# Desperodoo/distributed_multi_agent_reinforcement_learning

Hardware: AMD Instinct MI355X
Metric: env-steps/sec (whole node), pursuit-evasion 8-agent 4096-env (higher is better)
Workload: dtype f64 environment / f32 policy (f32 matrix products evaluated from exact 3-way bf16 operand splits, f32 accumulation and storage)

## Files before the change

### distributed_multi_agent_reinforcement_learning_amd/csrc/mappo_ops.hip

```cpp
#include <hip/hip_runtime.h>
#include <stdint.h>
#include <stdlib.h>
#include <string.h>

#include <mutex>

#include "mappo_ops.h"
#include "mappo_ops_diag.h"
#include "sb_common.hpp"
#include "sb_wgrad.hpp"
#include "ppo_diag.hpp"

namespace {

constexpr int MAX_P = 16;

__device__ __forceinline__ float msg_dot4(const float *w, const float4 &qv) {
    return __builtin_fmaf(w[3], qv.w, __builtin_fmaf(w[2], qv.z, __builtin_fmaf(w[1], qv.y, w[0] * qv.x)));
}

struct MsgDims {
    int R, P, K, E, din, q_div, adj_mode, rpb;
    int64_t p_rs, q_rs, e_rs, adj_rs, o_is;
};
// ... 2165 lines not shown
    if (pt == 4) MSGW3_PT(4) else if (pt == 8) MSGW3_PT(8) else MSGW3_PT(16)
#undef MSGW3_PT
#undef MSGW3_LAUNCH
#undef MSGW3_LAUNCH1
    return (int)hipGetLastError();
}

}

#include "gauss_policy.hpp"
#include "imitation.hpp"
#include "value_norm.hpp"
#include "fused_adam.hpp"

constexpr int SB_WGRAD_WGS = 256;

static bool sb_wgrad_shape_ok(int M, int N) {
    return (M == 128 || M == 256 || M == 384) && (N == 128 || N == 256 || N == 384) && M + N <= 512 && M * N < 256 * 256;
}

template <int MT, int NT>
int launch_sb_wgrad(int64_t K, const float *A, int64_t lda, const float *B, int64_t ldb, float *Cm, int accumulate, float *part, hipStream_t st,
                    const float *A2 = nullptr, int64_t lda2 = 0, int M1 = 0) {
    using C = SbWgCfg<MT, NT>;
    static std::once_flag once;
    static hipError_t attr_rc = hipSuccess;
    std::call_once(once, [] { attr_rc = hipFuncSetAttribute((const void *)k_sb_wgrad<MT, NT>, hipFuncAttributeMaxDynamicSharedMemorySize, C::LDS_BYTES); });
    if (attr_rc != hipSuccess) return (int)attr_rc;
    hipLaunchKernelGGL((k_sb_wgrad<MT, NT>), dim3(SB_WGRAD_WGS), dim3(SB_WG_THREADS), C::LDS_BYTES, st, A, lda, B, ldb, K, part, A2, lda2, M1);
    hipLaunchKernelGGL(k_wgrad_reduce, dim3((C::M * C::N + 63) / 64), dim3(256), 0, st, SB_WGRAD_WGS, C::M * C::N, (const float *)part, Cm, accumulate);
    return (int)hipGetLastError();
}

extern "C" {

int dhgn_msg_agg_fwd(int32_t R, int32_t P, int32_t K, int32_t E, int32_t din, const float *p, int64_t p_rs, const float *q,
                     int64_t q_rs, int32_t q_div, const float *e, int64_t e_rs, const void *adj, int64_t adj_rs, int32_t adj_mode,
                     const int32_t *kvalid, const float *W, const float *b, float *out, int64_t out_stride, void *stream) {
    int rc = check_msg(R, P, K, E, din, q_div, adj_mode, adj, kvalid, e);
    if (rc) return rc;
    if (R == 0) return 0;
    if ((q_rs & 3) || out_stride < E) return MO_ERR_BAD_ARG;
    int grid;
    const MsgDims d = msg_dims(R, P, K, E, din, q_div, adj_mode, p_rs, q_rs, e_rs, adj_rs, out_stride, FWD_BLOCKS, &grid);
    const bool qs = msg_q_small(K), as = msg_adj_small(P, K, adj_mode), ev2 = (E % 128) == 0;
#define MSGW_FWD1(PT, QS, AS, EV) hipLaunchKernelGGL((k_msgw_fwd<PT, QS, AS, EV>), dim3(grid), dim3(E / EV), 0, (hipStream_t)stream, d, p, q, e, adj, kvalid, W, b, out)
#define MSGW_FWD(PT, QS, AS) do { if (ev2) MSGW_FWD1(PT, QS, AS, 2); else MSGW_FWD1(PT, QS, AS, 1); } while (0)
#define MSGW_FWD_PT(PT) { if (qs && as) MSGW_FWD(PT, true, true); else if (qs) MSGW_FWD(PT, true, false); else if (as) MSGW_FWD(PT, false, true); else MSGW_FWD(PT, false, false); }
    if (P <= 8) MSGW_FWD_PT(8) else MSGW_FWD_PT(16)
#undef MSGW_FWD_PT
#undef MSGW_FWD
#undef MSGW_FWD1
    return (int)hipGetLastError();
}

int dhgn_msg_agg3_fwd(const mo_msg_rel *rel, int32_t R, int32_t P, int32_t E, const float *p, int64_t p_rs, float *out, int64_t out_stride,
                      void *stream) {
    if (!rel || !p || !out || R < 0) return MO_ERR_BAD_ARG;
    if (R == 0) return 0;
    return launch_msgw3(rel, R, P, E, p, p_rs, rel[2].kvalid, out, nullptr, 0, out_stride, stream, false);
}

int dhgn_msg_agg3_pair_fwd(const mo_msg_rel *rel, int32_t R, int32_t P, int32_t E, const float *p, int64_t p_rs, const int32_t *o_kvalid,
                           float *out_actor, float *out_critic, int64_t out_stride, void *stream) {
    if (!rel || !p || !out_actor || !out_critic || R < 0) return MO_ERR_BAD_ARG;
    if (R == 0) return 0;
// ... 340 lines not shown
}

int64_t wgrad_split_workspace(int32_t M, int32_t N) {
    if (!sb_wgrad_shape_ok(M, N)) return -1;
    return (int64_t)SB_WGRAD_WGS * M * N * sizeof(float);
}

int wgrad_split_tn(int64_t K, int32_t M, int32_t N, const float *A, int64_t lda, const float *B, int64_t ldb, float *C, int32_t accumulate,
                   void *workspace, void *stream) {
    if (K < 1 || !sb_wgrad_shape_ok(M, N) || !A || !B || !C || !workspace) return MO_ERR_BAD_ARG;
    if (lda < M || ldb < N || (lda & 3) || (ldb & 3) || ((uintptr_t)A & 15) || ((uintptr_t)B & 15)) return MO_ERR_BAD_ARG;
    hipStream_t st = (hipStream_t)stream;
    float *part = (float *)workspace;
#define SB_WG(mt, nt) if (M == 128 * mt && N == 128 * nt) return launch_sb_wgrad<mt, nt>(K, A, lda, B, ldb, C, accumulate, part, st);
    SB_WG(1, 1) SB_WG(1, 2) SB_WG(2, 1) SB_WG(1, 3) SB_WG(3, 1)
#undef SB_WG
    return MO_ERR_BAD_ARG;
}

int wgrad_split_tn2(int64_t K, int32_t M1, int32_t M2, int32_t N, const float *A1, int64_t lda1, const float *A2, int64_t lda2, const float *B, int64_t ldb,
                    float *C, int32_t accumulate, void *workspace, void *stream) {
    const int M = M1 + M2;
    if (K < 1 || M1 < 4 || M2 < 4 || (M1 & 3) || (M2 & 3) || !sb_wgrad_shape_ok(M, N) || !A1 || !A2 || !B || !C || !workspace) return MO_ERR_BAD_ARG;
    if (lda1 < M1 || lda2 < M2 || ldb < N || (lda1 & 3) || (lda2 & 3) || (ldb & 3) || ((uintptr_t)A1 & 15) || ((uintptr_t)A2 & 15) || ((uintptr_t)B & 15))
        return MO_ERR_BAD_ARG;
    hipStream_t st = (hipStream_t)stream;
    float *part = (float *)workspace;
#define SB_WG(mt, nt) if (M == 128 * mt && N == 128 * nt) return launch_sb_wgrad<mt, nt>(K, A1, lda1, B, ldb, C, accumulate, part, st, A2, lda2, M1);
    SB_WG(1, 1) SB_WG(1, 2) SB_WG(2, 1) SB_WG(1, 3) SB_WG(3, 1)
#undef SB_WG
    return MO_ERR_BAD_ARG;
}

int fcra_neighbour_mean(int32_t R, int32_t P, int32_t E, int32_t T, const float *z_actor, int64_t za_episode_stride, int64_t za_step_stride,
                        const float *z_critic, int64_t zc_episode_stride, int64_t zc_step_stride, const float *adj, int64_t adj_row_stride,
                        const float *bias, int32_t relu, float *out_actor, float *out_critic, int64_t out_stride, void *stream) {
    const mo_nbr_job job{z_actor, z_critic, bias, out_actor, out_critic};
    return fcra_neighbour_mean_multi(1, &job, R, P, E, T, za_episode_stride, za_step_stride, zc_episode_stride, zc_step_stride, adj, adj_row_stride, relu,
                                     out_stride, stream);
}

int fcra_neighbour_mean_multi(int32_t n_jobs, const mo_nbr_job *jobs, int32_t R, int32_t P, int32_t E, int32_t T, int64_t za_episode_stride,
                              int64_t za_step_stride, int64_t zc_episode_stride, int64_t zc_step_stride, const float *adj, int64_t adj_row_stride,
                              int32_t relu, int64_t out_stride, void *stream) {
    if (n_jobs < 1 || n_jobs > MO_NBR_MAX_JOBS || !jobs) return MO_ERR_BAD_ARG;
    if (R < 0 || P < 1 || P > MAX_P || E < 64 || E > 1024 || (E & 63) || T < 1 || (R % T) || out_stride < E) return MO_ERR_BAD_ARG;
    NbrJobs a_jobs;
    memset(&a_jobs, 0, sizeof a_jobs);
    for (int k = 0; k < n_jobs; k++) {
        const mo_nbr_job &m = jobs[k];
        if ((m.out_actor && (!m.z_actor || !adj)) || (m.out_critic && !m.z_critic) || (!m.out_actor && !m.out_critic)) return MO_ERR_BAD_ARG;
        a_jobs.j[k] = m;
    }
    if (R == 0) return 0;
    NbrArgs a{R, P, E, T, relu, za_episode_stride, za_step_stride, zc_episode_stride, zc_step_stride, adj_row_stride, out_stride};
    if (E == 128 && P <= 8 && !(out_stride & 3) && !(za_episode_stride & 3) && !(za_step_stride & 3) && !(zc_episode_stride & 3) && !(zc_step_stride & 3)) {
        bool aligned = true;
        for (int k = 0; k < n_jobs; k++) {
            const mo_nbr_job &m = jobs[k];
            aligned = aligned && !(((uintptr_t)m.z_actor | (uintptr_t)m.z_critic | (uintptr_t)m.bias | (uintptr_t)m.out_actor | (uintptr_t)m.out_critic) & 15);
        }
        if (aligned) {
            const int per4 = 4096 / n_jobs, blocks = (R + 3) / 4;
            hipLaunchKernelGGL(k_nbr_mean4, dim3(blocks < per4 ? blocks : per4, n_jobs), dim3(256), 0, (hipStream_t)stream, a, a_jobs, adj);
            return (int)hipGetLastError();
        }
// ... 178 lines not shown
```

### distributed_multi_agent_reinforcement_learning_amd/csrc/sb_wgrad.hpp

```cpp
#pragma once
#include "sb_common.hpp"

constexpr int SB_WG_MMA_WAVES = 8, SB_WG_LOAD_WAVES = 4, SB_WG_THREADS = 64 * (SB_WG_MMA_WAVES + SB_WG_LOAD_WAVES);

template <int MT, int NT>
struct SbWgCfg {
    static constexpr int M = 128 * MT, N = 128 * NT, COLS = M + N, FQ = COLS / 4;
    static constexpr int CR = 16, NO = 2;
    static constexpr int WGM = MT >= NT ? 4 : 2;
    static constexpr int WGN = 8 / WGM;
    static constexpr int TM = M / 32 / WGM, TN = N / 32 / WGN;
    static constexpr int UNITS = 2 * NO * FQ;
    static constexpr int LT = 64 * SB_WG_LOAD_WAVES;
    static constexpr int UL = (UNITS + LT - 1) / LT;
    static constexpr int DEPTH = UL == 1 ? 4 : 3;
    static constexpr int IMG = 3 * NO * COLS;
    static constexpr int LDS_BYTES = 2 * IMG * 16;
};

__device__ __forceinline__ int sb_swz(int f) { return (f & ~3) | ((f & 3) ^ ((f >> 3) & 3)); }

template <int MT, int NT>
__device__ __forceinline__ void sb_wgrad_loader(int lw, int lane, const float *__restrict__ A, int64_t lda, const float *__restrict__ B, int64_t ldb, int64_t K,
                                                const float *__restrict__ A2, int64_t lda2, int M1, int64_t c_beg, int64_t c_end, bool tail,
                                                uint4 *sb_lds) {
    using C = SbWgCfg<MT, NT>;
    const float *src[C::UL];
    int64_t ld[C::UL];
    bool on[C::UL];
    int row_in_chunk[C::UL], slot2[C::UL], sx[C::UL];
#pragma unroll
    for (int u = 0; u < C::UL; u++) {
        const int unit = 64 * lw + lane + C::LT * u;
        on[u] = (u + 1) * C::LT <= C::UNITS || 64 * lw + C::LT * u < C::UNITS;
        const int rest = on[u] ? unit / C::FQ : 0, col = on[u] ? 4 * (unit % C::FQ) : 0;
        row_in_chunk[u] = 4 * rest;
        const bool in_a2 = A2 != nullptr && col >= M1 && col < C::M;
        ld[u] = in_a2 ? lda2 : (col < C::M ? lda : ldb);
        src[u] = (in_a2 ? A2 + (col - M1) : (col < C::M ? A + col : B + (col - C::M))) + row_in_chunk[u] * ld[u];
        slot2[u] = 2 * ((rest >> 1) * C::COLS + col) + (rest & 1);
        sx[u] = (col >> 3) & 3;
    }
    constexpr int D = C::DEPTH;
    float4 raw[D][C::UL][4];
    auto fetch = [&](float4 (&r)[C::UL][4], int64_t c) {
        c = c < c_end ? c : c_end - 1;
#pragma unroll
        for (int u = 0; u < C::UL; u++) {
            const float *p = src[u] + c * C::CR * ld[u];
#pragma unroll
            for (int j = 0; j < 4; j++) r[u][j] = *(const float4 *)(p + j * ld[u]);
        }
    };
    auto stage = [&](const float4 (&r)[C::UL][4], uint4 *img) {
        uint2 *img2 = (uint2 *)img;
#pragma unroll
        for (int u = 0; u < C::UL; u++) {
            if (!on[u]) continue;
#pragma unroll
            for (int t = 0; t < 4; t++) {
                uint32_t p[3][2];
#pragma unroll
                for (int q = 0; q < 2; q++) {
                    const float4 &v0 = r[u][2 * q], &v1 = r[u][2 * q + 1];
                    const float x0 = t == 0 ? v0.x : t == 1 ? v0.y : t == 2 ? v0.z : v0.w;
                    const float x1 = t == 0 ? v1.x : t == 1 ? v1.y : t == 2 ? v1.z : v1.w;
                    sb_split2(x0, x1, p[0][q], p[1][q], p[2][q]);
                }
#pragma unroll
                for (int s = 0; s < 3; s++) img2[2 * s * C::NO * C::COLS + slot2[u] + 2 * (t ^ sx[u])] = make_uint2(p[s][0], p[s][1]);
            }
        }
    };
    if (c_beg < c_end) {
#pragma unroll
        for (int d = 0; d < D; d++) fetch(raw[d], c_beg + d);
        __builtin_amdgcn_sched_barrier(0);
        stage(raw[0], sb_lds);
        __builtin_amdgcn_sched_barrier(0);
        fetch(raw[0], c_beg + D);
    }
    lds_barrier();
    for (int64_t c = c_beg; c < c_end; c += D) {
#pragma unroll
        for (int d = 0; d < D; d++) {
            const int64_t cc = c + d;
            if (cc >= c_end) break;
            stage(raw[(d + 1) % D], sb_lds + ((cc + 1 - c_beg) & 1) * C::IMG);
            fetch(raw[(d + 1) % D], cc + 1 + D);
            lds_barrier();
        }
    }
    if (tail) {
        const int64_t r0 = (K / C::CR) * C::CR;
        float4 r[C::UL][4];
#pragma unroll
        for (int u = 0; u < C::UL; u++)
#pragma unroll
            for (int j = 0; j < 4; j++)
                r[u][j] = (on[u] && r0 + row_in_chunk[u] + j < K) ? *(const float4 *)(src[u] + (r0 + j) * ld[u]) : make_float4(0.f, 0.f, 0.f, 0.f);
        stage(r, sb_lds);
        lds_barrier();
    }
}

template <int MT, int NT>
__device__ __forceinline__ void sb_wgrad_mma(int wave, int lane, int64_t c_beg, int64_t c_end, bool tail, const uint4 *sb_lds, float *__restrict__ part) {
    using C = SbWgCfg<MT, NT>;
    const int i = lane & 31, g = lane >> 5;
    const int wm = wave / C::WGN, wn = wave % C::WGN;
    f32x16 acc[C::TM][C::TN];
#pragma unroll
    for (int a = 0; a < C::TM; a++)
#pragma unroll
        for (int b = 0; b < C::TN; b++)
#pragma unroll
            for (int r = 0; r < 16; r++) acc[a][b][r] = 0.f;
    auto multiply = [&](const uint4 *buf) {
        const uint4 *img = buf + g * C::COLS;
        constexpr int PS = C::NO * C::COLS;
        if constexpr (C::TN <= C::TM) {
            uint4 b[C::TN][3];
#pragma unroll
            for (int nt = 0; nt < C::TN; nt++) {
                const int f = sb_swz(C::M + 32 * (wn * C::TN + nt) + i);
#pragma unroll
                for (int s = 0; s < 3; s++) b[nt][s] = img[s * PS + f];
            }
#pragma unroll
            for (int mt = 0; mt < C::TM; mt++) {
                const int f = sb_swz(32 * (wm * C::TM + mt) + i);
                uint4 a[3];
#pragma unroll
// ... 23 lines not shown
    lds_barrier();
    for (int64_t c = c_beg; c < c_end; c++) {
        multiply(sb_lds + ((c - c_beg) & 1) * C::IMG);
        lds_barrier();
    }
    if (tail) {
        lds_barrier();
        multiply(sb_lds);
    }
    float *po = part + (size_t)blockIdx.x * C::M * C::N + (size_t)(32 * wm * C::TM + 4 * g) * C::N + 32 * wn * C::TN + i;
#pragma unroll
    for (int mt = 0; mt < C::TM; mt++)
#pragma unroll
        for (int r = 0; r < 16; r++)
#pragma unroll
            for (int nt = 0; nt < C::TN; nt++) po[(size_t)(32 * mt + 8 * (r / 4) + (r % 4)) * C::N + 32 * nt] = acc[mt][nt][r];
}

template <int MT, int NT>
__global__ __launch_bounds__(SB_WG_THREADS) void k_sb_wgrad(const float *__restrict__ A, int64_t lda, const float *__restrict__ B, int64_t ldb, int64_t K,
                                                            float *__restrict__ part, const float *__restrict__ A2, int64_t lda2, int M1) {
    using C = SbWgCfg<MT, NT>;
    static_assert(C::WGM * C::WGN == SB_WG_MMA_WAVES && C::TM * C::WGM * 32 == C::M && C::TN * C::WGN * 32 == C::N, "tiling");
    extern __shared__ uint4 sb_lds[];
    const int wave = __builtin_amdgcn_readfirstlane(threadIdx.x >> 6);
    const int64_t chunks = K / C::CR;
    const int64_t c_beg = chunks * blockIdx.x / gridDim.x, c_end = chunks * (blockIdx.x + 1) / gridDim.x;
    const bool tail = blockIdx.x == gridDim.x - 1 && (K % C::CR);
    if (wave >= SB_WG_MMA_WAVES)
        sb_wgrad_loader<MT, NT>(wave - SB_WG_MMA_WAVES, threadIdx.x & 63, A, lda, B, ldb, K, A2, lda2, M1, c_beg, c_end, tail, sb_lds);
    else
        sb_wgrad_mma<MT, NT>(wave, threadIdx.x & 63, c_beg, c_end, tail, sb_lds, part);
}
```

### distributed_multi_agent_reinforcement_learning_amd/ops.py

```python
import ctypes as C
import os

import torch
import torch.nn.functional as F

from . import build as _build

ADJ_TENSOR, ADJ_ONES, ADJ_VALID, ADJ_BITS = 0, 1, 2, 3
EXPORTS = ("dhgn_msg_agg_fwd", "dhgn_msg_agg3_fwd", "dhgn_msg_agg_bwd", "dhgn_msg_agg_bwd_workspace", "dhgn_msg_agg_ones_sorted_ok", "dhgn_msg_agg_ones_sorted_fwd",
           "dhgn_msg_agg_ones_sorted_bwd", "dhgn_msg_agg_ones_sorted_workspace", "gae_advnorm", "gae_advnorm_workspace", "categorical_sample",
           "categorical_sample_counter",
           "gru_gates_fwd", "gru_gates_bwd", "gru_cell_fwd", "gru_cell_fwd_multi", "gru_cell_split_fwd_multi", "sb_gemm_n128", "sb_gemm", "gru_seq_fwd", "gru_seq_fwd_multi", "gru_seq_split_fwd_multi", "gru_seq_split_bwd_multi", "gru_seq_save_elems", "gru_seq_bwd", "gru_seq_bwd_multi", "gru_seq_bwd_workspace", "wgrad_tn", "wgrad_tn_workspace", "wgrad_split_tn", "wgrad_split_tn2", "wgrad_split_workspace", "rollout_record", "ppo_loss_fwd_bwd", "ppo_loss_prob_fwd_bwd", "ppo_loss_workspace",
           "gauss_head_sample", "ppo_loss_gauss_fwd_bwd", "ppo_loss_gauss_workspace", "gauss_head_sample_ex", "ppo_loss_gauss_ex_fwd_bwd",
           "ppo_loss_gauss_ex_workspace", "gae_advnorm_vn", "gae_advnorm_vn_workspace", "value_norm_update", "value_norm_targets",
           "ppo_loss_fwd_bwd_diag", "ppo_loss_prob_fwd_bwd_diag", "ppo_loss_gauss_fwd_bwd_diag", "ppo_loss_gauss_ex_fwd_bwd_diag",
           "ppo_loss_diag_workspace", "ppo_loss_gauss_diag_workspace", "ppo_ratio", "ppo_diag_rows_host", "fused_adam_workspace",
           "fused_adam_grid", "fused_adam_norm", "fused_adam_step", "fused_adam_advance_host", "fused_adam_rows_host", "bc_loss_workspace",
           "bc_loss_gauss_fwd_bwd", "bc_loss_cat_fwd_bwd", "e3d_bc_select", "n2n_bc_select", "mappo_ops_error_string")

_lib = None


def lib_path():
    return _build.lib_path("libmappo_ops.so")


def load_library():
    global _lib
    if _lib is None:
        path = lib_path()
        if not os.path.exists(path):
            raise RuntimeError(f"{path} is missing: build it with __graft_entry__.build() (hipcc --offload-arch=gfx950); "
                               "the fused MAPPO ops have no fallback")
        L = C.CDLL(path)
        vp, i32, i64, f32, f64 = C.c_void_p, C.c_int32, C.c_int64, C.c_float, C.c_double
        L.dhgn_msg_agg_fwd.argtypes = [i32, i32, i32, i32, i32, vp, i64, vp, i64, i32, vp, i64, vp, i64, i32, vp, vp, vp, vp, i64, vp]
        L.dhgn_msg_agg_bwd.argtypes = [i32, i32, i32, i32, i32, vp, i64, vp, i64, i32, vp, i64, vp, i64, i32, vp, vp, vp, vp, i64, vp, vp, vp, vp]
        L.dhgn_msg_agg3_fwd.argtypes = [vp, i32, i32, i32, vp, i64, vp, i64, vp]
        L.dhgn_msg_agg3_pair_fwd.argtypes = [vp, i32, i32, i32, vp, i64, vp, vp, vp, i64, vp]
        L.dhgn_msg_agg3_pair01_fwd.argtypes = [vp, i32, i32, i32, vp, i64, vp, vp, i64, vp]
        L.dhgn_msg_agg_bwd_pair.argtypes = [i32, i32, i32, i32, i32, vp, i64, vp, i64, i32, vp, i64, vp, i64, vp, vp, vp, vp, i64, vp, vp, vp, vp]
        L.dhgn_msg_agg3_pair_pos_fwd.argtypes = [vp, i32, i32, i32, vp, i64, vp, vp, vp, i64, vp, i64, vp, vp, vp, i64, vp]
        L.spectral_norm_weight.argtypes = [i32, i32, vp, vp, vp, f32, i32, vp, vp]
        L.dhgn_msg_agg_bwd_workspace.argtypes = [i32, i32]
        L.dhgn_msg_agg_bwd_workspace.restype = i64
# ... 6 lines not shown
        L.gae_advnorm_workspace.restype = i64
        L.gae_advnorm_vn.argtypes = [i32, i32, i32, vp, vp, vp, vp, vp, f32, f32, i32, vp, vp, vp, vp, vp]
        L.gae_advnorm_vn_workspace.restype = i64
        L.value_norm_update.argtypes = [vp, vp, C.c_double, vp]
        L.value_norm_targets.argtypes = [i64, vp, vp, vp, vp, vp]
        L.categorical_sample.argtypes = [i32, i32, vp, C.c_uint64, C.c_uint64, i32, vp, vp, vp]
        L.categorical_sample_counter.argtypes = [i32, i32, vp, C.c_uint64, vp, i32, vp, vp, vp]
        L.head_linear.argtypes = [i32, i32, i32, vp, vp, vp, vp, vp]
        L.head_sample.argtypes = [i32, i32, i32, vp, vp, vp, C.c_uint64, vp, vp, i32, vp, vp, vp]
        L.gru_gates_fwd.argtypes = [i32, i32, vp, vp, vp, vp, vp, vp, vp]
        L.gru_gates_bwd.argtypes = [i32, i32, vp, vp, vp, vp, vp, vp, vp, vp]
        L.gru_cell_fwd.argtypes = [i32, i32, vp, vp, vp, vp, vp, vp, vp, vp]
        L.gru_seq_fwd.argtypes = [i32, i32, i32, vp, vp, vp, vp, vp, vp, i32, vp]
        L.gru_seq_bwd.argtypes = [i32, i32, i32, vp, vp, vp, vp, vp, vp, vp, vp, vp, vp, vp, i32, vp, vp]
        L.gru_cell_fwd_multi.argtypes = [i32, vp, i32, i32, vp]
        L.gru_cell_split_fwd_multi.argtypes = [i32, vp, i32, i32, vp]
        L.sb_gemm_n128.argtypes = [i64, i32, vp, i64, vp, i64, vp, i32, vp, i64, vp, i64, vp]
        L.sb_gemm.argtypes = [i64, i32, i32, vp, i64, vp, i64, vp, i32, vp, i64, vp, i64, vp]
        L.gru_seq_fwd_multi.argtypes = [i32, vp, i32, i32, i32, i32, vp]
        L.gru_seq_bwd_multi.argtypes = [i32, vp, i32, i32, i32, i32, vp]
        L.gru_seq_split_fwd_multi.argtypes = [i32, vp, i32, i32, i32, i32, vp]
        L.gru_seq_split_bwd_multi.argtypes = [i32, vp, i32, i32, i32, i32, vp]
        L.gru_seq_save_elems.argtypes = [i32, i32]
        L.gru_seq_save_elems.restype = i64
        L.gru_seq_bwd_workspace.argtypes = [i32]
        L.gru_seq_bwd_workspace.restype = i64
        L.wgrad_tn_workspace.argtypes = [i32, i32]
        L.wgrad_tn_workspace.restype = i64
        L.wgrad_tn.argtypes = [i64, i32, i32, vp, i64, vp, i64, vp, i32, vp, vp]
        L.wgrad_split_workspace.restype = i64
        L.wgrad_split_workspace.argtypes = [i32, i32]
        L.wgrad_split_tn.argtypes = [i64, i32, i32, vp, i64, vp, i64, vp, i32, vp, vp]
        L.wgrad_split_tn2.argtypes = [i64, i32, i32, i32, vp, i64, vp, i64, vp, i64, vp, i32, vp, vp]
        L.fcra_neighbour_mean.argtypes = [i32, i32, i32, i32, vp, i64, i64, vp, i64, i64, vp, i64, vp, i32, vp, vp, i64, vp]
        L.fcra_neighbour_mean_multi.argtypes = [i32, vp, i32, i32, i32, i32, i64, i64, i64, i64, vp, i64, i32, i64, vp]
        L.sb_gemm_signs.argtypes = [i64, i32, i32, vp, i64, vp, i64, vp, i32, vp, i64, vp, i64, vp, i64, vp]
        L.sb_gemm_masked_bits.argtypes = [i64, i32, i32, vp, i64, vp, i64, vp, i64, i32, vp, i64, vp, vp, vp]
        L.sb_gemm_masked_workspace.argtypes = [i32]
        L.sb_gemm_masked_workspace.restype = i64
        L.sb_gemm_masked.argtypes = [i64, i32, i32, vp, i64, vp, i64, vp, i64, i32, vp, i64, vp, vp, vp]
        L.relu_bwd_colsum_workspace.argtypes = [i32]
        L.relu_bwd_colsum_workspace.restype = i64
        L.relu_bwd_colsum.argtypes = [i64, i32, vp, i64, vp, i64, vp, vp, vp, vp]
        L.wgrad_skinny_workspace.argtypes = [i32, i32]
        L.wgrad_skinny_workspace.restype = i64
        L.wgrad_skinny.argtypes = [i64, i32, i32, vp, i64, vp, i64, i32, vp, vp, vp, vp, vp]
        L.rollout_record.argtypes = [i32, i32, vp, vp, vp, i32, vp]
        L.ppo_loss_workspace.restype = i64
        L.ppo_loss_fwd_bwd.argtypes = [i64, vp, vp, vp, vp, vp, vp, vp, vp, vp, f32, f32, i32, vp, vp, vp, vp, vp, vp]
        L.ppo_loss_prob_fwd_bwd.argtypes = [i64, i32, vp, vp, i64, i64, i64, i64, i64, vp, vp, vp, vp, vp, i64, i64, i64, vp, vp, vp, f32, f32, i32, vp, vp, vp, vp]
        L.gauss_head_sample.argtypes = [i32, i32, i32, vp, vp, vp, vp, C.c_uint64, vp, vp, i32, vp, vp, vp, vp]
        L.ppo_loss_gauss_workspace.restype = i64
        L.ppo_loss_gauss_fwd_bwd.argtypes = [i64, i32, vp, vp, i64, i64, i64, i64, i64, vp, vp, vp, vp, vp, vp, i64, i64, i64, vp, vp, vp, f32, f32,
                                             i32, vp, vp, vp, vp, vp]
        L.gauss_head_sample_ex.argtypes = [i32, i32, i32, vp, vp, vp, vp, vp, vp, f32, f32, i32, C.c_uint64, vp, vp, i32, vp, vp, vp, vp]
        L.ppo_loss_gauss_ex_workspace.restype = i64
        L.ppo_loss_gauss_ex_fwd_bwd.argtypes = [i64, i32, vp, vp, i64, i64, i64, i64, i64, vp, vp, i64, i64, i64, f32, f32, i32, vp, vp, vp, vp,
                                                vp, i64, i64, i64, vp, vp, vp, f32, f32, i32, vp, vp, vp, vp]
        for name in ("ppo_loss_fwd_bwd", "ppo_loss_prob_fwd_bwd", "ppo_loss_gauss_fwd_bwd", "ppo_loss_gauss_ex_fwd_bwd"):
            getattr(L, name + "_diag").argtypes = getattr(L, name).argtypes + [vp]
        L.ppo_loss_diag_workspace.restype = i64
        L.ppo_loss_gauss_diag_workspace.restype = i64
        L.ppo_ratio.argtypes = [i64, vp, vp, vp, vp, vp]
        L.ppo_diag_rows_host.argtypes = [i64, vp, vp, vp, vp, vp, vp, f32, vp]
        L.fused_adam_workspace.restype = i64
        L.fused_adam_grid.argtypes = [i64]
# ... 1345 lines not shown
    _need_gpu(logp_now, "ppo_ratio")
    a, b = logp_now.contiguous(), logp_old.contiguous()
    assert a.dtype == b.dtype == torch.float32 and a.shape == b.shape
    lr, ratio = torch.empty_like(a), torch.empty_like(a)
    _check(L.ppo_ratio(a.numel(), _ptr(a), _ptr(b), _ptr(lr), _ptr(ratio), _stream()), "ppo_ratio")
    return lr, ratio


class RecordItem(C.Structure):
    _fields_ = [("src", C.c_void_p), ("dst", C.c_void_p), ("dst_row_stride", C.c_int64), ("row_bytes", C.c_int32), ("i32_to_f32", C.c_int32)]


def rollout_record(pairs, raw=None, episode_return=None):
    L = load_library()
    n = len(pairs)
    arr = (RecordItem * max(n, 1))()
    N = pairs[0][0].shape[0]
    for k, (src, dst) in enumerate(pairs):
        _need_gpu(src, "rollout_record")
        assert src.is_contiguous() and src.shape == dst.shape and src.shape[0] == N and (N == 1 or dst[0].is_contiguous())
        conv = src.dtype == torch.int32 and dst.dtype == torch.float32
        assert conv or src.dtype == dst.dtype
        it = arr[k]
        it.src, it.dst = src.data_ptr(), dst.data_ptr()
        it.row_bytes = src[0].numel() * src.element_size()
        it.dst_row_stride = dst.stride(0) * dst.element_size()
        it.i32_to_f32 = int(conv)
    P = raw.shape[1] if raw is not None else 0
    _check(L.rollout_record(N, n, C.cast(arr, C.c_void_p), _ptr(raw), _ptr(episode_return), P, _stream()), "rollout_record")


PERSISTENT_GRU_MIN_T = 2
SEQ_MODE = os.environ.get("MAPPO_GRU_SEQ", os.environ.get("MAPPO_MATMUL", "split_bf16"))


def _seq_fwd(L, arr, n, T, Bmax, H, agents):
    if SEQ_MODE == "split_bf16":
        _check(L.gru_seq_split_fwd_multi(n, C.cast(arr, C.c_void_p), T, Bmax, H, agents, _stream()), "gru_seq_split_fwd_multi")
    else:
        _check(L.gru_seq_fwd_multi(n, C.cast(arr, C.c_void_p), T, Bmax, H, agents, _stream()), "gru_seq_fwd_multi")


def _seq_bwd(L, arr, n, T, Bmax, H, agents):
    if SEQ_MODE == "split_bf16":
        _check(L.gru_seq_split_bwd_multi(n, C.cast(arr, C.c_void_p), T, Bmax, H, agents, _stream()), "gru_seq_split_bwd_multi")
    else:
        _check(L.gru_seq_bwd_multi(n, C.cast(arr, C.c_void_p), T, Bmax, H, agents, _stream()), "gru_seq_bwd_multi")


class _GRULayer(torch.autograd.Function):

    @staticmethod
    def forward(ctx, x, h0, w_ih, w_hh, b_ih, b_hh, T, B, agents):
        L = load_library()
        _need_gpu(x, "gru")
        I = x.shape[-1]
        H = w_hh.shape[1]
        persistent = bool(H == 128 and T >= PERSISTENT_GRU_MIN_T)
        ctx.x_shape = x.shape
        ctx.ungather = 0
        if agents and not persistent:
            x = x.reshape(B // agents, T, agents, I).permute(1, 0, 2, 3).reshape(T, B, I)
            ctx.ungather = int(agents)
            agents = 0
        x = x.contiguous()
        h0 = h0.contiguous()
# ... 13 lines not shown
            a = arr[0]
            a.gi, a.w_hh, a.b_hh, a.h0, a.out = gi.data_ptr(), whh.data_ptr(), b_hh.data_ptr(), h0.data_ptr(), out.data_ptr()
            a.save = save.data_ptr() if need else None
            a.B = B
            _seq_fwd(L, arr, 1, T, B, H, int(agents))
            if need:
                ctx.save_for_backward(x, h0, w_ih, whh, out, save)
            return out
        gi = gi.reshape(T, B, 3 * H)
        gh = torch.empty((B, 3 * H), dtype=x.dtype, device=x.device)
        w_hh_t = w_hh.t()
        hprev = h0
        for t in range(T):
            torch.mm(hprev, w_hh_t, out=gh)
            _check(L.gru_gates_fwd(B, H, _ptr(gi[t]), _ptr(gh), _ptr(b_hh), _ptr(hprev), _ptr(out[t]),
                                   _ptr(save[t]) if need else None, st), "gru_gates_fwd")
            hprev = out[t]
        if need:
            ctx.save_for_backward(x, h0, w_ih, w_hh, out, save)
        return out

    @staticmethod
    def backward(ctx, dout):
        L = load_library()
        x, h0, w_ih, w_hh, out, save = ctx.saved_tensors
        T, B, I = ctx.dims
        H = w_hh.shape[1]
        dout = dout.contiguous()
        dgi = torch.empty((T * B, 3 * H), dtype=x.dtype, device=x.device)
        dh_direct = torch.empty((B, H), dtype=x.dtype, device=x.device)
        dcarry = None
        st = _stream()
        db_ih = db_hh = None
        split = bool(ctx.persistent and not ctx.agents)
        dgh = None if split else torch.empty((T, B, 3 * H), dtype=x.dtype, device=x.device)
        dnr = torch.empty((T, B, H), dtype=x.dtype, device=x.device) if split else None
        if ctx.persistent:
            db_ih = torch.empty(3 * H, dtype=x.dtype, device=x.device)
            db_hh = torch.empty(3 * H, dtype=x.dtype, device=x.device)
            ws = torch.empty(L.gru_seq_bwd_workspace(B), dtype=torch.uint8, device=x.device)
            arr = (GruSeqBwdNet * 1)()
            a = arr[0]
            a.dout, a.save, a.out, a.h0, a.w_hh, a.dgi = dout.data_ptr(), save.data_ptr(), out.data_ptr(), h0.data_ptr(), w_hh.data_ptr(), dgi.data_ptr()
            a.dgh = dgh.data_ptr() if dgh is not None else None
            a.dnr = dnr.data_ptr() if dnr is not None else None
            a.dh0, a.db_ih, a.db_hh, a.workspace = dh_direct.data_ptr(), db_ih.data_ptr(), db_hh.data_ptr(), ws.data_ptr()
            a.B = B
            _seq_bwd(L, arr, 1, T, B, H, ctx.agents)
            dcarry = dh_direct
        else:
            dgi3 = dgi.view(T, B, 3 * H)
            for t in range(T - 1, -1, -1):
                hprev = out[t - 1] if t > 0 else h0
                _check(L.gru_gates_bwd(B, H, _ptr(dout[t]), _ptr(dcarry), _ptr(save[t]), _ptr(hprev), _ptr(dgi3[t]), _ptr(dgh[t]),
                                       _ptr(dh_direct), st), "gru_gates_bwd")
                dcarry = torch.addmm(dh_direct, dgh[t], w_hh)
        dw_hh = _gru_dw_hh(dgi, dgh, dnr, out, h0, T, B, H)
        x2 = x.reshape(T * B, I)
        dw_ih = wgrad(dgi, x2)
        dx = None
        if ctx.needs_input_grad[0]:
            dx = input_grad(dgi, w_ih)
            if ctx.ungather:
                P = ctx.ungather
                dx = dx.reshape(T, B // P, P, I).permute(1, 0, 2, 3)
            dx = dx.reshape(ctx.x_shape)
        if db_ih is None:
            db_ih, db_hh = dgi.sum(0), dgh.reshape(T * B, 3 * H).sum(0)
        return dx, dcarry, dw_ih, dw_hh, db_ih, db_hh, None, None, None


class GruCellNet(C.Structure):
    _fields_ = [(n, C.c_void_p) for n in ("x", "h_prev", "w_ih", "w_hh", "b_ih", "b_hh", "h_out")]


CELL_MODE = os.environ.get("MAPPO_GRU_CELL", MATMUL_MODE)


def set_cell_mode(mode):
    global CELL_MODE
    if mode not in ("fp32", "split_bf16"):
        raise ValueError(f"matmul mode {mode!r}: 'fp32' or 'split_bf16'")
    CELL_MODE = mode


def matmul_modes():
    return MATMUL_MODE, WGRAD_MODE, PROJ_MODE, CELL_MODE, SEQ_MODE


def restore_matmul_modes(modes):
# ... 112 lines not shown
        arr = (GruSeqNet * n)()
        keep = []
        for k in range(n):
            x, h0, w_ih, w_hh, b_ih, b_hh = ts[6 * k: 6 * k + 6]
            _need_gpu(x, "gru")
            I, B = x.shape[-1], Bs[k]
            x, h0 = x.contiguous(), h0.contiguous()
            out = torch.empty((T, B, H), dtype=x.dtype, device=x.device)
            gi = gru_input_projection(x.reshape(T * B, I), w_ih, b_ih)
            save = torch.empty(L.gru_seq_save_elems(T, B), dtype=x.dtype, device=x.device) if need else None
            whh, bhh = w_hh.detach().contiguous(), b_hh.detach().contiguous()
            a = arr[k]
            a.gi, a.w_hh, a.b_hh, a.h0, a.out = gi.data_ptr(), whh.data_ptr(), bhh.data_ptr(), h0.data_ptr(), out.data_ptr()
            a.save = save.data_ptr() if need else None
            a.B = B
            keep.append((gi, whh, bhh))
            outs.append(out)
            saved += [x, h0, w_ih, whh, out, save]
        _seq_fwd(L, arr, n, T, max(Bs), H, int(agents))
        ctx.dims, ctx.agents, ctx.n = (T, tuple(Bs)), int(agents), n
        ctx.x_links, ctx.zero_h0 = x_links, bool(zero_h0)
        ctx.x_shapes = [ts[6 * k].shape for k in range(n)]
        if need:
            ctx.save_for_backward(*saved)
        return tuple(outs)

    @staticmethod
    def backward(ctx, *douts):
        L = load_library()
        T, Bs = ctx.dims
        n = ctx.n
        sv = ctx.saved_tensors
        H = 128
        split = not ctx.agents
        arr = (GruSeqBwdNet * n)()
        per = []
        for k in range(n):
            x, h0, w_ih, w_hh, out, save = sv[6 * k: 6 * k + 6]
            dev, dt, B = x.device, x.dtype, Bs[k]
            dout = douts[k].contiguous()
            dgi = torch.empty((T * B, 3 * H), dtype=dt, device=dev)
            dgh = None if split else torch.empty((T, B, 3 * H), dtype=dt, device=dev)
            dnr = torch.empty((T, B, H), dtype=dt, device=dev) if split else None
            dh0 = torch.empty((B, H), dtype=dt, device=dev)
            db_ih, db_hh = torch.empty(3 * H, dtype=dt, device=dev), torch.empty(3 * H, dtype=dt, device=dev)
            ws = torch.empty(L.gru_seq_bwd_workspace(B), dtype=torch.uint8, device=dev)
            a = arr[k]
            a.dout, a.save, a.out, a.h0, a.w_hh, a.dgi = dout.data_ptr(), save.data_ptr(), out.data_ptr(), h0.data_ptr(), w_hh.data_ptr(), dgi.data_ptr()
            a.dgh = dgh.data_ptr() if dgh is not None else None
            a.dnr = dnr.data_ptr() if dnr is not None else None
            a.dh0, a.db_ih, a.db_hh, a.workspace = dh0.data_ptr(), db_ih.data_ptr(), db_hh.data_ptr(), ws.data_ptr()
            a.B = B
            per.append((dout, dgi, dgh, dnr, dh0, db_ih, db_hh, ws))
        _seq_bwd(L, arr, n, T, max(Bs), H, ctx.agents)
        grads = [None, None, None, None, None]
        for k in range(n):
            x, h0, w_ih, w_hh, out, save = sv[6 * k: 6 * k + 6]
            dout, dgi, dgh, dnr, dh0, db_ih, db_hh, ws = per[k]
            B = Bs[k]
            dw_hh = _gru_dw_hh(dgi, dgh, dnr, out, h0, T, B, H, ctx.zero_h0)
            I = x.shape[-1]
            x2 = x.reshape(T * B, I)
            dw_ih = wgrad(dgi, x2)
            dx = None
            if ctx.needs_input_grad[5 + 6 * k]:
                link = ctx.x_links[k] if ctx.x_links is not None else None
                fused = input_grad_masked(dgi, w_ih, x2, I, link.bits) if link is not None else None
                if fused is not None:
                    dx, link.db = fused
                else:
                    dx = input_grad(dgi, w_ih)
                dx = dx.reshape(ctx.x_shapes[k])
            grads += [dx, dh0, dw_ih, dw_hh, db_ih, db_hh]
        return tuple(grads)


def _gru_dw_hh(dgi, dgh, dnr, out, h0, T, B, H, zero_h0=False):
    if dgh is not None:
        dw_hh = torch.mm(dgh[0].t(), h0)
        if T > 1:
            wgrad(dgh[1:].reshape((T - 1) * B, 3 * H), out[:-1].reshape((T - 1) * B, H), out=dw_hh, accumulate=True)
        return dw_hh
    dw_hh = torch.empty((3 * H, H), dtype=dgi.dtype, device=dgi.device)
    drz, hp = dgi[:, :2 * H], out[:-1].reshape((T - 1) * B, H)
    acc = True
    if zero_h0 and T > 1:
        acc = False
    elif zero_h0:
        dw_hh.zero_()
    else:
        torch.mm(drz[:B].t(), h0, out=dw_hh[:2 * H])
        torch.mm(dnr[0].t(), h0, out=dw_hh[2 * H:])
    if T > 1:
        a1, a2 = drz[B:], dnr[1:].reshape((T - 1) * B, H)
        if WGRAD_MODE == "split_bf16" and H == 128 and _wgrad_ok(a1, hp) and _wgrad_ok(a2, hp):
            L = load_library()
            ws = torch.empty(L.wgrad_split_workspace(3 * H, H), dtype=torch.uint8, device=dgi.device)
            _check(L.wgrad_split_tn2(a1.shape[0], 2 * H, H, H, _ptr(a1), a1.stride(0), _ptr(a2), a2.stride(0), _ptr(hp), hp.stride(0), _ptr(dw_hh), int(acc),
                                     _ptr(ws), _stream()), "wgrad_split_tn2")
        else:
            wgrad(a1, hp, out=dw_hh[:2 * H], accumulate=acc)
            wgrad(a2, hp, out=dw_hh[2 * H:], accumulate=acc)
    return dw_hh


def gru_multi(xs, h0s, modules, agents=0, steps=None, grouped=False, x_links=None, zero_state=False):
    n = len(xs)
    if agents:
        assert xs[0].dim() == 2 and steps and all(x.shape[0] % (steps * agents) == 0 for x in xs)
        T, Bs = int(steps), [x.shape[0] // int(steps) for x in xs]
    else:
        T, Bs = xs[0].shape[0], [x.shape[1] for x in xs]
    tiles = sum((B + 15) // 16 for B in Bs)
    ok = (n <= GRU_MULTI_MAX_NETS and T >= PERSISTENT_GRU_MIN_T and all(x.shape[-1] == xs[0].shape[-1] and x.dim() == xs[0].dim() for x in xs)
          and (grouped or (tiles <= GRU_MULTI_MAX_WORKGROUPS and all(B == Bs[0] for B in Bs)))
          and all(m.num_layers == modules[0].num_layers and m.weight_hh_l0.shape == (384, 128) for m in modules))
# ... 39 lines not shown
```

### include/mappo_ops.h

```cpp
#ifndef MAPPO_OPS_H
#define MAPPO_OPS_H
#include <stdint.h>

#ifdef __cplusplus
extern "C" {
#endif

#define MO_ERR_BAD_ARG 20001

enum { MO_ADJ_TENSOR = 0,
       MO_ADJ_ONES = 1,
       MO_ADJ_VALID = 2,
       MO_ADJ_BITS = 3 };
#define MO_ADJ_ROW_WORDS(K) (((((K) + 31) >> 5) + 3) & ~3)

int dhgn_msg_agg_fwd(int32_t R, int32_t P, int32_t K, int32_t E, int32_t din, const float *p, int64_t p_row_stride,
                     const float *q, int64_t q_row_stride, int32_t q_div, const float *e, int64_t e_row_stride, const void *adj,
                     int64_t adj_row_stride, int32_t adj_mode, const int32_t *kvalid, const float *W, const float *b,
                     float *out, int64_t out_stride , void *stream);

typedef struct mo_msg_rel {
    int32_t K, din, q_div, adj_mode;
    const float *q; int64_t q_rs;
    const float *e; int64_t e_rs;
// ... 165 lines not shown

int64_t bc_loss_workspace(void);
int bc_loss_gauss_fwd_bwd(int64_t n, int32_t A, const float *mu, float *grad_mu, int64_t d1, int64_t d2, int64_t m_s0, int64_t m_s1, int64_t m_s2,
                          const float *ls_raw, float *grad_log_std, int64_t l_s0, int64_t l_s1, int64_t l_s2, float log_std_min, float log_std_max,
                          int32_t fit_std, int32_t wrap0, const float *target, const float *active, const float *values_now, int64_t v_s0,
                          int64_t v_s1, int64_t v_s2, const float *values_old, const float *v_target, const float *active_sum, float epsilon,
                          int32_t use_value_clip, float *losses, float *grad_values, double *sums, void *workspace, void *stream);
int bc_loss_cat_fwd_bwd(int64_t n, int32_t A, const float *prob, float *grad_prob, int64_t d1, int64_t d2, int64_t p_s0, int64_t p_s1, int64_t p_s2,
                        const float *label, const float *active, const float *values_now, int64_t v_s0, int64_t v_s1, int64_t v_s2,
                        const float *values_old, const float *v_target, const float *active_sum, float epsilon, int32_t use_value_clip,
                        float *losses, float *grad_values, double *sums, void *workspace, void *stream);
int e3d_bc_select(int32_t N, int32_t P, const double *guide, const uint8_t *follow, int32_t squash, double bound, double *env_action, float *a_star,
                  int64_t row_stride, void *stream);
int n2n_bc_select(int32_t N, int32_t P, const int32_t *guide, const uint8_t *follow, int32_t *a_n, float *a_star, int64_t row_stride, void *stream);

#define MO_RECORD_MAX_ITEMS 16
typedef struct {
    const void *src;
    void *dst;
    int64_t dst_row_stride;
    int32_t row_bytes;
    int32_t i32_to_f32;
} mo_record_item;
int rollout_record(int32_t N, int32_t n_items, const mo_record_item *items, const float *raw, float *episode_return, int32_t P, void *stream);

int64_t wgrad_tn_workspace(int32_t M, int32_t N);
int wgrad_tn(int64_t K, int32_t M, int32_t N, const float *A, int64_t lda, const float *B, int64_t ldb, float *C, int32_t accumulate,
             void *workspace, void *stream);
int64_t wgrad_split_workspace(int32_t M, int32_t N);
int wgrad_split_tn(int64_t K, int32_t M, int32_t N, const float *A, int64_t lda, const float *B, int64_t ldb, float *C, int32_t accumulate,
                   void *workspace, void *stream);
int wgrad_split_tn2(int64_t K, int32_t M1, int32_t M2, int32_t N, const float *A1, int64_t lda1, const float *A2, int64_t lda2, const float *B, int64_t ldb,
                    float *C, int32_t accumulate, void *workspace, void *stream);
int fcra_neighbour_mean(int32_t R, int32_t P, int32_t E, int32_t T, const float *z_actor, int64_t za_episode_stride, int64_t za_step_stride,
                        const float *z_critic, int64_t zc_episode_stride, int64_t zc_step_stride, const float *adj, int64_t adj_row_stride,
                        const float *bias, int32_t relu, float *out_actor, float *out_critic, int64_t out_stride, void *stream);
#define MO_NBR_MAX_JOBS 4
typedef struct mo_nbr_job { const float *z_actor, *z_critic, *bias; float *out_actor, *out_critic; } mo_nbr_job;
int fcra_neighbour_mean_multi(int32_t n_jobs, const mo_nbr_job *jobs, int32_t R, int32_t P, int32_t E, int32_t T, int64_t za_episode_stride,
                              int64_t za_step_stride, int64_t zc_episode_stride, int64_t zc_step_stride, const float *adj, int64_t adj_row_stride,
                              int32_t relu, int64_t out_stride, void *stream);

int64_t relu_bwd_colsum_workspace(int32_t F);
int relu_bwd_colsum(int64_t R, int32_t F, const float *gout, int64_t g_row_stride, const float *y, int64_t y_row_stride, float *gin, float *colsum,
                    void *workspace, void *stream);

int64_t wgrad_skinny_workspace(int32_t NS, int32_t F);
int wgrad_skinny(int64_t R, int32_t NS, int32_t F, const float *S, int64_t lds, const float *X, int64_t ldx, int32_t transposed, float *C,
                 float *colsum_x, float *colsum_s, void *workspace, void *stream);

const char *mappo_ops_error_string(int code);

#ifdef __cplusplus
}
#endif
#endif
```

Baseline: 2.647 million.

## Add index-mapped split wgrad for GRU hidden weights with agent-major gate gradients

Adds a specialised wgrad kernel for the GRU hidden-to-hidden weight gradient whose loader remaps rows, so dgi stored in (episode, time, agent) order can be read directly. Before, agent-structured GRUs fell back to materialising a full dgh tensor and computing dw_hh from it. Now the persistent split path with dnr is used, and the separate gradient buffer plus its reductions are avoided. The cost is per-row index arithmetic in the loader and strided, less contiguous loads.

```diff
diff --git a/distributed_multi_agent_reinforcement_learning_amd/csrc/mappo_ops.hip b/distributed_multi_agent_reinforcement_learning_amd/csrc/mappo_ops.hip
--- a/distributed_multi_agent_reinforcement_learning_amd/csrc/mappo_ops.hip
+++ b/distributed_multi_agent_reinforcement_learning_amd/csrc/mappo_ops.hip
@@ -2221,6 +2221,18 @@
     return (int)hipGetLastError();
 }
 
+static int launch_sb_wgrad_gru_hh(int T, int B, int agents, const float *dgi, const float *dnr, const float *out, float *Cm, int accumulate, float *part,
+                           hipStream_t st) {
+    using C = SbWgCfg<3, 1>;
+    static std::once_flag once;
+    static hipError_t attr_rc = hipSuccess;
+    std::call_once(once, [] { attr_rc = hipFuncSetAttribute((const void *)k_sb_wgrad_gru_hh, hipFuncAttributeMaxDynamicSharedMemorySize, C::LDS_BYTES); });
+    if (attr_rc != hipSuccess) return (int)attr_rc;
+    hipLaunchKernelGGL(k_sb_wgrad_gru_hh, dim3(SB_WGRAD_WGS), dim3(SB_WG_THREADS), C::LDS_BYTES, st, dgi, dnr + (size_t)B * C::N, out, SbWgMap{T, B, agents}, part);
+    hipLaunchKernelGGL(k_wgrad_reduce, dim3((C::M * C::N + 63) / 64), dim3(256), 0, st, SB_WGRAD_WGS, C::M * C::N, (const float *)part, Cm, accumulate);
+    return (int)hipGetLastError();
+}
+
 extern "C" {
 
 int dhgn_msg_agg_fwd(int32_t R, int32_t P, int32_t K, int32_t E, int32_t din, const float *p, int64_t p_rs, const float *q,
@@ -2627,6 +2639,13 @@
     return MO_ERR_BAD_ARG;
 }
 
+int wgrad_split_gru_hh(int32_t T, int32_t B, int32_t agents, const float *dgi, const float *dnr, const float *out, float *C, int32_t accumulate,
+                       void *workspace, void *stream) {
+    if (T < 2 || B < 4 || agents < 4 || (B & 3) || (agents & 3) || B % agents || (int64_t)T * B > INT32_MAX) return MO_ERR_BAD_ARG;
+    if (!dgi || !dnr || !out || !C || !workspace || ((uintptr_t)dgi & 15) || ((uintptr_t)dnr & 15) || ((uintptr_t)out & 15)) return MO_ERR_BAD_ARG;
+    return launch_sb_wgrad_gru_hh(T, B, agents, dgi, dnr, out, C, accumulate, (float *)workspace, (hipStream_t)stream);
+}
+
 int fcra_neighbour_mean(int32_t R, int32_t P, int32_t E, int32_t T, const float *z_actor, int64_t za_episode_stride, int64_t za_step_stride,
                         const float *z_critic, int64_t zc_episode_stride, int64_t zc_step_stride, const float *adj, int64_t adj_row_stride,
                         const float *bias, int32_t relu, float *out_actor, float *out_critic, int64_t out_stride, void *stream) {
diff --git a/distributed_multi_agent_reinforcement_learning_amd/csrc/sb_wgrad.hpp b/distributed_multi_agent_reinforcement_learning_amd/csrc/sb_wgrad.hpp
--- a/distributed_multi_agent_reinforcement_learning_amd/csrc/sb_wgrad.hpp
+++ b/distributed_multi_agent_reinforcement_learning_amd/csrc/sb_wgrad.hpp
@@ -18,13 +18,16 @@
     static constexpr int LDS_BYTES = 2 * IMG * 16;
 };
 
+struct SbWgMap { int T, B, P; };
+
 __device__ __forceinline__ int sb_swz(int f) { return (f & ~3) | ((f & 3) ^ ((f >> 3) & 3)); }
 
-template <int MT, int NT>
+template <int MT, int NT, bool MAP = false>
 __device__ __forceinline__ void sb_wgrad_loader(int lw, int lane, const float *__restrict__ A, int64_t lda, const float *__restrict__ B, int64_t ldb, int64_t K,
                                                 const float *__restrict__ A2, int64_t lda2, int M1, int64_t c_beg, int64_t c_end, bool tail,
-                                                uint4 *sb_lds) {
+                                                uint4 *sb_lds, SbWgMap map = SbWgMap{0, 1, 1}) {
     using C = SbWgCfg<MT, NT>;
+    static_assert(!MAP || (C::FQ % 64 == 0 && C::UNITS % C::LT == 0), "MAP: a loader wave's units share their row, and none is idle");
     const float *src[C::UL];
     int64_t ld[C::UL];
     bool on[C::UL];
@@ -41,13 +44,39 @@
         slot2[u] = 2 * ((rest >> 1) * C::COLS + col) + (rest & 1);
         sx[u] = (col >> 3) & 3;
     }
+    [[maybe_unused]] bool mapped = false;
+    [[maybe_unused]] int m_t[C::UL], m_e[C::UL], m_p[C::UL], adv_t = 0, adv_e = 0, adv_p = 0, m_eb = 1;
+    if constexpr (MAP) {
+        mapped = 4 * ((64 * lw) % C::FQ) < M1;
+        m_eb = map.B / map.P;
+        adv_t = C::CR / map.B;
+        adv_e = (C::CR % map.B) / map.P;
+        adv_p = (C::CR % map.B) % map.P;
+#pragma unroll
+        for (int u = 0; u < C::UL; u++) {
+            const uint32_t r = (uint32_t)c_beg * C::CR + 4 * ((64 * lw + C::LT * u) / C::FQ), b = r % (uint32_t)map.B;
+            m_t[u] = (int)(r / (uint32_t)map.B) + 1;
+            m_e[u] = (int)(b / (uint32_t)map.P);
+            m_p[u] = (int)(b % (uint32_t)map.P);
+            if (mapped) src[u] -= row_in_chunk[u] * ld[u];
+        }
+    }
     constexpr int D = C::DEPTH;
     float4 raw[D][C::UL][4];
     auto fetch = [&](float4 (&r)[C::UL][4], int64_t c) {
+        [[maybe_unused]] const bool advance = c + 1 < c_end;
         c = c < c_end ? c : c_end - 1;
 #pragma unroll
         for (int u = 0; u < C::UL; u++) {
             const float *p = src[u] + c * C::CR * ld[u];
+            if constexpr (MAP) {
+                const int row = (m_e[u] * map.T + m_t[u]) * map.P + m_p[u];
+                p = mapped ? src[u] + (int64_t)row * ld[u] : p;
+                int t = m_t[u] + adv_t, e = m_e[u] + adv_e, a = m_p[u] + adv_p;
+                if (a >= map.P) { a -= map.P; e++; }
+                if (e >= m_eb) { e -= m_eb; t++; }
+                m_t[u] = advance ? t : m_t[u]; m_e[u] = advance ? e : m_e[u]; m_p[u] = advance ? a : m_p[u];
+            }
 #pragma unroll
             for (int j = 0; j < 4; j++) r[u][j] = *(const float4 *)(p + j * ld[u]);
         }
@@ -95,10 +124,17 @@
         const int64_t r0 = (K / C::CR) * C::CR;
         float4 r[C::UL][4];
 #pragma unroll
-        for (int u = 0; u < C::UL; u++)
+        for (int u = 0; u < C::UL; u++) {
+            const float *p = src[u] + r0 * ld[u];
+            if constexpr (MAP) {
+                const uint32_t rr = (uint32_t)r0 + 4 * ((64 * lw + C::LT * u) / C::FQ), b = rr % (uint32_t)map.B;
+                const int row = ((int)(b / (uint32_t)map.P) * map.T + (int)(rr / (uint32_t)map.B) + 1) * map.P + (int)(b % (uint32_t)map.P);
+                p = mapped ? src[u] + (int64_t)row * ld[u] : p;
+            }
 #pragma unroll
             for (int j = 0; j < 4; j++)
-                r[u][j] = (on[u] && r0 + row_in_chunk[u] + j < K) ? *(const float4 *)(src[u] + (r0 + j) * ld[u]) : make_float4(0.f, 0.f, 0.f, 0.f);
+                r[u][j] = (on[u] && r0 + row_in_chunk[u] + j < K) ? *(const float4 *)(p + j * ld[u]) : make_float4(0.f, 0.f, 0.f, 0.f);
+        }
         stage(r, sb_lds);
         lds_barrier();
     }
@@ -188,3 +224,18 @@
     else
         sb_wgrad_mma<MT, NT>(wave, threadIdx.x & 63, c_beg, c_end, tail, sb_lds, part);
 }
+
+__global__ __launch_bounds__(SB_WG_THREADS) void k_sb_wgrad_gru_hh(const float *__restrict__ dgi, const float *__restrict__ dnr1,
+                                                                   const float *__restrict__ hprev, SbWgMap map, float *__restrict__ part) {
+    using C = SbWgCfg<3, 1>;
+    extern __shared__ uint4 sb_lds[];
+    const int wave = __builtin_amdgcn_readfirstlane(threadIdx.x >> 6);
+    const int64_t K = (int64_t)(map.T - 1) * map.B;
+    const int64_t chunks = K / C::CR;
+    const int64_t c_beg = chunks * blockIdx.x / gridDim.x, c_end = chunks * (blockIdx.x + 1) / gridDim.x;
+    const bool tail = blockIdx.x == gridDim.x - 1 && (K % C::CR);
+    if (wave >= SB_WG_MMA_WAVES)
+        sb_wgrad_loader<3, 1, true>(wave - SB_WG_MMA_WAVES, threadIdx.x & 63, dgi, C::M, hprev, C::N, K, dnr1, C::N, 256, c_beg, c_end, tail, sb_lds, map);
+    else
+        sb_wgrad_mma<3, 1>(wave, threadIdx.x & 63, c_beg, c_end, tail, sb_lds, part);
+}
diff --git a/distributed_multi_agent_reinforcement_learning_amd/ops.py b/distributed_multi_agent_reinforcement_learning_amd/ops.py
--- a/distributed_multi_agent_reinforcement_learning_amd/ops.py
+++ b/distributed_multi_agent_reinforcement_learning_amd/ops.py
@@ -10,7 +10,7 @@
 EXPORTS = ("dhgn_msg_agg_fwd", "dhgn_msg_agg3_fwd", "dhgn_msg_agg_bwd", "dhgn_msg_agg_bwd_workspace", "dhgn_msg_agg_ones_sorted_ok", "dhgn_msg_agg_ones_sorted_fwd",
            "dhgn_msg_agg_ones_sorted_bwd", "dhgn_msg_agg_ones_sorted_workspace", "gae_advnorm", "gae_advnorm_workspace", "categorical_sample",
            "categorical_sample_counter",
-           "gru_gates_fwd", "gru_gates_bwd", "gru_cell_fwd", "gru_cell_fwd_multi", "gru_cell_split_fwd_multi", "sb_gemm_n128", "sb_gemm", "gru_seq_fwd", "gru_seq_fwd_multi", "gru_seq_split_fwd_multi", "gru_seq_split_bwd_multi", "gru_seq_save_elems", "gru_seq_bwd", "gru_seq_bwd_multi", "gru_seq_bwd_workspace", "wgrad_tn", "wgrad_tn_workspace", "wgrad_split_tn", "wgrad_split_tn2", "wgrad_split_workspace", "rollout_record", "ppo_loss_fwd_bwd", "ppo_loss_prob_fwd_bwd", "ppo_loss_workspace",
+           "gru_gates_fwd", "gru_gates_bwd", "gru_cell_fwd", "gru_cell_fwd_multi", "gru_cell_split_fwd_multi", "sb_gemm_n128", "sb_gemm", "gru_seq_fwd", "gru_seq_fwd_multi", "gru_seq_split_fwd_multi", "gru_seq_split_bwd_multi", "gru_seq_save_elems", "gru_seq_bwd", "gru_seq_bwd_multi", "gru_seq_bwd_workspace", "wgrad_tn", "wgrad_tn_workspace", "wgrad_split_tn", "wgrad_split_tn2", "wgrad_split_gru_hh", "wgrad_split_workspace", "rollout_record", "ppo_loss_fwd_bwd", "ppo_loss_prob_fwd_bwd", "ppo_loss_workspace",
            "gauss_head_sample", "ppo_loss_gauss_fwd_bwd", "ppo_loss_gauss_workspace", "gauss_head_sample_ex", "ppo_loss_gauss_ex_fwd_bwd",
            "ppo_loss_gauss_ex_workspace", "gae_advnorm_vn", "gae_advnorm_vn_workspace", "value_norm_update", "value_norm_targets",
            "ppo_loss_fwd_bwd_diag", "ppo_loss_prob_fwd_bwd_diag", "ppo_loss_gauss_fwd_bwd_diag", "ppo_loss_gauss_ex_fwd_bwd_diag",
@@ -83,6 +83,7 @@
         L.wgrad_split_workspace.argtypes = [i32, i32]
         L.wgrad_split_tn.argtypes = [i64, i32, i32, vp, i64, vp, i64, vp, i32, vp, vp]
         L.wgrad_split_tn2.argtypes = [i64, i32, i32, i32, vp, i64, vp, i64, vp, i64, vp, i32, vp, vp]
+        L.wgrad_split_gru_hh.argtypes = [i32, i32, i32, vp, vp, vp, vp, i32, vp, vp]
         L.fcra_neighbour_mean.argtypes = [i32, i32, i32, i32, vp, i64, i64, vp, i64, i64, vp, i64, vp, i32, vp, vp, i64, vp]
         L.fcra_neighbour_mean_multi.argtypes = [i32, vp, i32, i32, i32, i32, i64, i64, i64, i64, vp, i64, i32, i64, vp]
         L.sb_gemm_signs.argtypes = [i64, i32, i32, vp, i64, vp, i64, vp, i32, vp, i64, vp, i64, vp, i64, vp]
@@ -1494,6 +1495,12 @@
 
 PERSISTENT_GRU_MIN_T = 2
 SEQ_MODE = os.environ.get("MAPPO_GRU_SEQ", os.environ.get("MAPPO_MATMUL", "split_bf16"))
+GRU_HH_MAP = os.environ.get("MAPPO_GRU_HH_MAP", "1") != "0"
+
+
+def _gru_hh_map_ok(T, B, H, agents):
+    return bool(GRU_HH_MAP and agents and SEQ_MODE == "split_bf16" and WGRAD_MODE == "split_bf16" and H == 128 and T >= 2
+                and B % 4 == 0 and agents % 4 == 0 and B % agents == 0 and (T - 1) * B >= WGRAD_MIN_ROWS and T * B < 2 ** 31)
 
 
 def _seq_fwd(L, arr, n, T, Bmax, H, agents):
@@ -1573,7 +1580,8 @@
         dcarry = None
         st = _stream()
         db_ih = db_hh = None
-        split = bool(ctx.persistent and not ctx.agents)
+        mapped = bool(ctx.persistent and _gru_hh_map_ok(T, B, H, ctx.agents))
+        split = bool(ctx.persistent and (not ctx.agents or mapped))
         dgh = None if split else torch.empty((T, B, 3 * H), dtype=x.dtype, device=x.device)
         dnr = torch.empty((T, B, H), dtype=x.dtype, device=x.device) if split else None
         if ctx.persistent:
@@ -1596,7 +1604,7 @@
                 _check(L.gru_gates_bwd(B, H, _ptr(dout[t]), _ptr(dcarry), _ptr(save[t]), _ptr(hprev), _ptr(dgi3[t]), _ptr(dgh[t]),
                                        _ptr(dh_direct), st), "gru_gates_bwd")
                 dcarry = torch.addmm(dh_direct, dgh[t], w_hh)
-        dw_hh = _gru_dw_hh(dgi, dgh, dnr, out, h0, T, B, H)
+        dw_hh = _gru_dw_hh(dgi, dgh, dnr, out, h0, T, B, H, agents=ctx.agents if mapped else 0)
         x2 = x.reshape(T * B, I)
         dw_ih = wgrad(dgi, x2)
         dx = None
@@ -1775,7 +1783,8 @@
         n = ctx.n
         sv = ctx.saved_tensors
         H = 128
-        split = not ctx.agents
+        mapped = all(_gru_hh_map_ok(T, B, H, ctx.agents) for B in Bs)
+        split = not ctx.agents or mapped
         arr = (GruSeqBwdNet * n)()
         per = []
         for k in range(n):
@@ -1801,7 +1810,7 @@
             x, h0, w_ih, w_hh, out, save = sv[6 * k: 6 * k + 6]
             dout, dgi, dgh, dnr, dh0, db_ih, db_hh, ws = per[k]
             B = Bs[k]
-            dw_hh = _gru_dw_hh(dgi, dgh, dnr, out, h0, T, B, H, ctx.zero_h0)
+            dw_hh = _gru_dw_hh(dgi, dgh, dnr, out, h0, T, B, H, ctx.zero_h0, agents=ctx.agents if mapped else 0)
             I = x.shape[-1]
             x2 = x.reshape(T * B, I)
             dw_ih = wgrad(dgi, x2)
@@ -1818,13 +1827,22 @@
         return tuple(grads)
 
 
-def _gru_dw_hh(dgi, dgh, dnr, out, h0, T, B, H, zero_h0=False):
+def _gru_dw_hh(dgi, dgh, dnr, out, h0, T, B, H, zero_h0=False, agents=0):
     if dgh is not None:
         dw_hh = torch.mm(dgh[0].t(), h0)
         if T > 1:
             wgrad(dgh[1:].reshape((T - 1) * B, 3 * H), out[:-1].reshape((T - 1) * B, H), out=dw_hh, accumulate=True)
         return dw_hh
     dw_hh = torch.empty((3 * H, H), dtype=dgi.dtype, device=dgi.device)
+    if agents:
+        L = load_library()
+        if not zero_h0:
+            drz0 = dgi.view(B // agents, T, agents, 3 * H)[:, 0, :, :2 * H].reshape(B, 2 * H)
+            torch.mm(torch.cat((drz0, dnr[0]), dim=1).t(), h0, out=dw_hh)
+        ws = torch.empty(L.wgrad_split_workspace(3 * H, H), dtype=torch.uint8, device=dgi.device)
+        _check(L.wgrad_split_gru_hh(T, B, agents, _ptr(dgi), _ptr(dnr), _ptr(out), _ptr(dw_hh), int(not zero_h0), _ptr(ws), _stream()),
+               "wgrad_split_gru_hh")
+        return dw_hh
     drz, hp = dgi[:, :2 * H], out[:-1].reshape((T - 1) * B, H)
     acc = True
     if zero_h0 and T > 1:
diff --git a/include/mappo_ops.h b/include/mappo_ops.h
--- a/include/mappo_ops.h
+++ b/include/mappo_ops.h
@@ -221,6 +221,8 @@
                    void *workspace, void *stream);
 int wgrad_split_tn2(int64_t K, int32_t M1, int32_t M2, int32_t N, const float *A1, int64_t lda1, const float *A2, int64_t lda2, const float *B, int64_t ldb,
                     float *C, int32_t accumulate, void *workspace, void *stream);
+int wgrad_split_gru_hh(int32_t T, int32_t B, int32_t agents, const float *dgi, const float *dnr, const float *out, float *C, int32_t accumulate,
+                       void *workspace, void *stream);
 int fcra_neighbour_mean(int32_t R, int32_t P, int32_t E, int32_t T, const float *z_actor, int64_t za_episode_stride, int64_t za_step_stride,
                         const float *z_critic, int64_t zc_episode_stride, int64_t zc_step_stride, const float *adj, int64_t adj_row_stride,
                         const float *bias, int32_t relu, float *out_actor, float *out_critic, int64_t out_stride, void *stream);
```

Result: no change. 2.671 million (median of 6 runs) (+0.9%).
